# ChristianFeldmann/libHM

Measured on AMD Instinct MI355X. Metric: decoded Mpixels/s (luma), 2160p Main10 reconstruction + loop filters, higher is better.
Workload: dtype int16 samples / int32 accumulate; 1 GPU; 3840x2160 Main10 lowdelay_P pictures, pre-parsed CTU metadata: prep+MC+dequant/IT/recon+deblock+SAO, batch of 16 independent pictures per step, inputs resident in HBM; sub_benchmark=full, streams=2, parallelism=frame-parallel, 1 process per GPU, no data-path collective

## Files before the change

### libhm_amd/csrc/hmgpu_api.hip

```cpp
#include "hmgpu_dev.h"
#include "packed_format.h"

#include <algorithm>
#include <chrono>
#include <atomic>
#include <cstdio>
#include <cstring>
#include <cstdlib>
#include <new>
#include <thread>
#include <unordered_map>
#include <vector>

using namespace hmgpu;

namespace {

enum { K_PREP = 0, K_MC_LUMA, K_MC_CHROMA, K_ITX, K_DBK_VER, K_DBK_HOR, K_SAO, K_EXTEND, K_H2D, K_INTRA, K_FILTER, K_UNPACK };
const char* const kKernelNames[HMGPU_NUM_KERNELS] = {"prep", "mc_luma", "mc_chroma", "itx", "deblock_ver", "deblock_hor", "sao",
                                                     "extend_border", "h2d_stage", "intra", "filter_fused", "unpack"};

struct SliceCall { int first_ctu, num_ctus, slice_idx; bool intra, wp, cells, bi, islice; };

struct Picture {
  bool in_use = false;
  bool sao_applied = false;
  bool filter_ready = false;
  bool sao_any = false;
  bool extended = false;
  std::vector<SliceCall> calls;
  void* planes = nullptr;
  void* meta = nullptr;
  void* coef = nullptr;
  void* pcm = nullptr;
  void* ccp = nullptr;
  void* blob = nullptr;
  void* derived = nullptr;
  uint8_t* sl_table = nullptr;
  uint32_t* coef_start = nullptr;
  std::vector<uint8_t> sl_host;
  PicDev dev;
  std::vector<SliceDev> slices;
  std::vector<SaoDev> h_saoprm;
  std::vector<uint16_t> h_slice_idx, h_tile_idx;
  int max_slice = -1;
  bool flags_staged = true;
  uint64_t last_use = 0;
};

struct EventPair { hipEvent_t a, b; int kind; };

}
// ... 213 lines not shown
    Carver m(pass ? p.meta : nullptr);
    carve_meta(m, p.dev, np, c->num_ctus);
    if (!pass) { HIP_TRY(c, hipMalloc(&p.meta, m.off)); HIP_TRY(c, hipMemset(p.meta, 0, m.off)); }
  }
  {
    size_t bytes = 0;
    for (int k = 0; k < 3; k++) bytes += align_up(c->coef_elems[k] * sizeof(int16_t), 256);
    HIP_TRY(c, hipMalloc(&p.coef, bytes));
    HIP_TRY(c, hipMemset(p.coef, 0, bytes));
    Carver m(p.coef);
    for (int k = 0; k < 3; k++) p.dev.coef[k] = m.take<int16_t>(c->coef_elems[k]);
  }
  for (int pass = 0; pass < 2; pass++) {
    Carver m(pass ? p.derived : nullptr);
    PicDev& d = p.dev;
    d.blk = m.take<BlkInfo>((size_t)c->grid_w * c->grid_h);
    d.edges = m.take<EdgeRec>((size_t)(c->grid_w / 2) * (c->grid_h / 2));
    d.tmv = m.take<TileMv>((size_t)(c->grid_w / 2) * (c->grid_h / 2));
    for (int k = 0; k < 3; k++) d.resid[k] = m.take<int16_t>(c->coef_elems[k]);
    for (int k = 0; k < 3; k++) d.quad_off[k] = m.take<uint32_t>((size_t)c->num_ctus * (c->parts / 4));
    p.coef_start = m.take<uint32_t>((size_t)3 * (c->num_ctus + 1));
    d.fault = m.take<uint32_t>(1);
    for (int k = 0; k < 4; k++) d.tu[k] = m.take<TuRec>((size_t)c->tu_cap[k] * kTuShards);
    d.tu_count = m.take<uint32_t>(4 * kTuShards);
    d.stats = m.take<unsigned long long>(2 * kTuShards);
    d.saoprm = m.take<SaoDev>((size_t)c->num_ctus * 3);
    d.slices = m.take<SliceDev>(HMGPU_MAX_SLICES);
    d.ctu_intra = m.take<uint8_t>((size_t)c->num_ctus);
    p.sl_table = m.take<uint8_t>(4 * 6 * 1024);
    d.intra_done = m.take<uint32_t>((size_t)3 * c->num_ctus);
    if (!pass) { HIP_TRY(c, hipMalloc(&p.derived, m.off)); HIP_TRY(c, hipMemset(p.derived, 0, m.off)); }
  }
  PicDev& d = p.dev;
  d.width = s.width; d.height = s.height;
  d.bd[0] = s.bit_depth_luma; d.bd[1] = d.bd[2] = s.bit_depth_chroma;
  d.log2ctu = s.log2_ctu_size; d.ctus_w = c->ctus_w; d.ctus_h = c->ctus_h; d.num_ctus = c->num_ctus; d.parts = c->parts; d.pw = c->pw;
  for (int k = 0; k < 3; k++) d.pitch[k] = c->pitch[k];
  d.grid_w = c->grid_w; d.grid_h = c->grid_h;
  d.lf_across_tiles = 1; d.sao_applied = 0;
  d.has_intra_dir = 0; d.strong_intra_smoothing = s.strong_intra_smoothing ? 1 : 0;
  d.range_ext = s.range_ext_flags;
  d.mono = s.chroma_format == 0 ? 1 : 0;
  d.fmt = c->fmt; d.csx = c->csx; d.csy = c->csy;
  d.ccp[0] = d.ccp[1] = nullptr;
  d.debug_skip_ctu = -1;
  d.sl_m = nullptr;
  for (int k = 0; k < 3; k++) { d.pcm[k] = nullptr; d.pcm_shift[k] = 0; d.coef_start[k] = nullptr; }
// ... 44 lines not shown
  if (p.extended) return HMGPU_OK;
  Batch b; memset(&b, 0, sizeof(b));
  b.n = 1; b.pic[0] = pic;
  { ProfScope ps(c, K_EXTEND); launch_extend(c->d_pics, b, c->seq.width, c->seq.height, c->mx[0], c->my[0], c->csx, c->csy, c->stream); }
  HIP_TRY(c, hipGetLastError());
  p.extended = true;
  return HMGPU_OK;
}
hmgpu_status ensure_refs_extended(hmgpu_ctx* c, const Batch& b, size_t call_idx) {
  for (int i = 0; i < b.n; i++) {
    const Picture& p = c->pics[b.pic[i]];
    if (call_idx >= p.calls.size()) continue;
    const SliceDev& sd = p.slices[p.calls[call_idx].slice_idx];
    for (int l = 0; l < 2; l++)
      for (int r = 0; r < HMGPU_MAX_REF; r++)
        if (sd.ref_pic[l][r] >= 0) { hmgpu_status st = ensure_extended(c, sd.ref_pic[l][r]); if (st != HMGPU_OK) return st; }
  }
  return HMGPU_OK;
}

hmgpu_status run_recon(hmgpu_ctx* c, const Batch& b, bool any_intra, bool any_wp, bool any_cells, bool any_bi, bool any_islice) {
  int max_ctus = 0;
  for (int i = 0; i < b.n; i++) max_ctus = std::max(max_ctus, b.num_ctus[i]);
  { ProfScope ps(c, K_PREP); launch_prep(c->d_pics, b, max_ctus, c->parts, any_intra, any_cells || c->fmt != 1, c->fmt, c->stream); }
  if (c->fmt != 1) {
    for (int i = 0; i < b.n; i++) {
      const PicDev& d = c->pics[b.pic[i]].dev;
      HIP_TRY(c, hipMemsetAsync(d.resid[1], 0, (size_t)((char*)d.resid[2] - (char*)d.resid[1]) + c->coef_elems[2] * sizeof(int16_t), c->stream));
    }
  }
  McArgs ma;
  memset(&ma, 0, sizeof(ma));
  ma.n = b.n; ma.width = c->seq.width; ma.height = c->seq.height; ma.log2ctu = c->seq.log2_ctu_size; ma.ctus_w = c->ctus_w;
  ma.tw = c->grid_w / 2; ma.npics = c->seq.max_pictures;
  ma.slab = c->plane_slab; ma.pic_stride = 2 * c->plane_bytes; ma.slab_bytes = ma.pic_stride * c->pics.size(); ma.sao_off = (uint32_t)c->plane_bytes;
  for (size_t i = 0; i < c->pics.size(); i++)
    if (c->pics[i].sao_applied) (i < 32 ? ma.sao_mask_lo : ma.sao_mask_hi) |= 1u << (i & 31);
  for (int i = 0; i < b.n; i++) {
    const PicDev& d = c->pics[b.pic[i]].dev;
    ma.first_ctu[i] = b.first_ctu[i]; ma.num_ctus[i] = b.num_ctus[i];
    ma.tmv[i] = d.tmv; ma.slices[i] = d.slices;
  }
  const PicDev& d0 = c->pics[b.pic[0]].dev;
  const char* const base0 = (const char*)c->pics[b.pic[0]].planes;
  uint32_t bps = (uint32_t)std::max(4, std::min(b.n >= 4 ? 12 : 24, max_ctus / 8 + 1));
  {
    ItxArgs ia;
    memset(&ia, 0, sizeof(ia));
    ia.n = b.n; ia.class_mask = 0xf;
    for (int k = 0; k < 3; k++) { ia.rtw[k] = (c->grid_w / 2) >> (k ? c->csx : 0); ia.bd[k] = d0.bd[k]; }
    ia.csx = c->csx; ia.csy = c->csy;
    for (int k = 0; k < 4; k++) ia.tu_cap[k] = c->tu_cap[k];
    for (int i = 0; i < b.n; i++) {
      const PicDev& d = c->pics[b.pic[i]].dev;
      for (int k = 0; k < 4; k++) ia.tu[i][k] = d.tu[k];
      ia.tu_count[i] = d.tu_count;
      for (int k = 0; k < 3; k++) { ia.coef[i][k] = d.coef[k]; ia.resid[i][k] = d.resid[k]; }
      ia.sl_m[i] = d.sl_m;
    }
    ProfScope ps(c, K_ITX);
    launch_itx(ia, bps, c->stream);
    bool any_ccp = false;
    for (int i = 0; i < b.n; i++) any_ccp |= c->pics[b.pic[i]].dev.ccp[0] != nullptr;
    if (any_ccp) launch_ccp(c->d_pics, b, max_ctus, c->stream);
  }
  {
    ProfScope ps(c, K_MC_LUMA);
    ma.pitch = c->pitch[0]; ma.bd = c->seq.bit_depth_luma;
    ma.origin_off = (uint32_t)((const char*)d0.rec[0] - base0);
    ma.rtw = c->grid_w / 2;
    for (int i = 0; i < b.n; i++) { ma.dst[i] = c->pics[b.pic[i]].dev.rec[0]; ma.resid[i] = c->pics[b.pic[i]].dev.resid[0]; }
    launch_mc_luma(ma, max_ctus, any_wp, any_bi, c->stream);
    if (any_cells) launch_mc_luma_cells(c->d_pics, c->d_finals, b, max_ctus, c->seq.log2_ctu_size, any_wp, c->stream);
  }
  if (c->fmt != 1) {
    ProfScope ps(c, K_MC_CHROMA);
    launch_mc_chroma_fmt(c->d_pics, c->d_finals, b, max_ctus, c->seq.log2_ctu_size, c->fmt, any_wp, c->stream);
  } else if (c->seq.chroma_format != 0) {
    ProfScope ps(c, K_MC_CHROMA);
// ... 1568 lines not shown
```

### libhm_amd/csrc/hmgpu_dev.h

```cpp
#pragma once
#include <hip/hip_runtime.h>
#include <stdint.h>
#include "../../include/hmgpu.h"

namespace hmgpu {

constexpr int kMaxBatch = 16;
constexpr int kMaxPics = 64;
constexpr int kTuShards = 8;
constexpr int kCStep = 2;

struct __attribute__((aligned(16))) BlkInfo {
  int16_t mv[2][2];
  int8_t  ref[2];
  int8_t  qp;
  uint8_t flags;
  uint8_t edge;
  uint8_t log2cu;
  uint16_t slice;
};
static_assert(sizeof(BlkInfo) == 16, "BlkInfo must be 16 bytes");

enum : uint8_t {
  BF_VALID = 1,
// ... 131 lines not shown
  const SliceDev* slices[kMaxBatch];
  const char* slab;
  uint64_t pic_stride, slab_bytes;
  uint32_t sao_off, origin_off, cr_off;
  uint32_t sao_mask_lo, sao_mask_hi;
};

struct ItxArgs {
  int32_t n; uint32_t class_mask;
  int32_t blocks[4];
  int32_t rtw[3], bd[3];
  int32_t csx, csy;
  uint32_t tu_cap[4];
  const TuRec* tu[kMaxBatch][4];
  const uint32_t* tu_count[kMaxBatch];
  const int16_t* coef[kMaxBatch][3];
  int16_t* resid[kMaxBatch][3];
  const uint8_t* sl_m[kMaxBatch];
};

#define HMGPU_AS1 __attribute__((address_space(1)))
typedef uint32_t u32x4 __attribute__((ext_vector_type(4)));
typedef uint32_t u32x2 __attribute__((ext_vector_type(2)));
typedef u32x4 u32x4_a8 __attribute__((aligned(8)));
template <typename T> __device__ inline T ldg(const T* p) { return *(const T HMGPU_AS1*)p; }
template <typename T> __device__ inline void stg(T* p, T v) { *(T HMGPU_AS1*)p = v; }
__device__ inline u32x4 ldg4(const void* p) { return *(const u32x4 HMGPU_AS1*)p; }
__device__ inline u32x4 ldg4_a8(const void* p) { return *(const u32x4_a8 HMGPU_AS1*)p; }
__device__ inline u32x2 ldg2(const void* p) { return *(const u32x2 HMGPU_AS1*)p; }
__device__ inline void stg4(void* p, u32x4 v) { *(u32x4 HMGPU_AS1*)p = v; }
__device__ inline void stg4_a8(void* p, u32x4 v) { *(u32x4_a8 HMGPU_AS1*)p = v; }
__device__ inline void stg2(void* p, u32x2 v) { *(u32x2 HMGPU_AS1*)p = v; }

__host__ __device__ inline int zscan_x(int z) {
  int x = z & 0x5555; x = (x | (x >> 1)) & 0x3333; x = (x | (x >> 2)) & 0x0f0f; x = (x | (x >> 4)) & 0x00ff; return x;
}
__host__ __device__ inline int zscan_y(int z) { return zscan_x(z >> 1); }
__device__ inline int clip3(int lo, int hi, int v) { return min(hi, max(lo, v)); }
__device__ inline BlkInfo ld_blk(const BlkInfo* p) { return __builtin_bit_cast(BlkInfo, ldg4(p)); }

__device__ inline bool xcd_remap(int bid, int n, int nb, int& slot, int& lb) {
  if (n < 0) { n = -n; slot = bid % n; lb = bid / n; return lb < nb; }
  if (n <= 8 && (8 % n) == 0) {
    const int m = 8 / n;
    const int per = (nb + m - 1) / m;
    const int x = bid & 7, t = bid >> 3;
    slot = x % n;
    const int r = x / n;
    lb = r * per + t;
    return t < per && lb < nb;
  }
  slot = bid % n; lb = bid / n;
  return lb < nb;
}
__host__ inline int xcd_grid(int n, int nb) {
  if (n <= 8 && (8 % n) == 0) { const int m = 8 / n; return 8 * ((nb + m - 1) / m); }
  return n * nb;
}

struct UnpackArgs {
  int32_t n;
  int32_t pic[kMaxBatch];
  const char* blob[kMaxBatch];
};
void launch_unpack_input(const PicDev* pics, const UnpackArgs& ua, int num_ctus, hipStream_t s);
void launch_prep(const PicDev* pics, const Batch& b, int max_ctus, int parts, bool intra, bool write_blk, int fmt, hipStream_t s);
void launch_mc_luma(McArgs& a, int max_ctus, bool wp, bool bi, hipStream_t s);
void launch_mc_chroma(McArgs& a, int max_ctus, bool wp, bool bi, hipStream_t s);
void launch_mc_luma_cells(const PicDev* pics, const PlaneSet* finals, const Batch& b, int max_ctus, int log2ctu, bool wp, hipStream_t s);
void launch_mc_chroma_cells(const PicDev* pics, const PlaneSet* finals, const Batch& b, int max_ctus, int log2ctu, bool wp, hipStream_t s);
void launch_itx(ItxArgs& a, uint32_t blocks_per_shard, hipStream_t s);
void launch_filter_fused(const PicDev* pics, const Batch& b, int width, int height, bool nofilt, hipStream_t s);
void launch_pack(const int16_t* src, int pitch, int step, int x0, int y0, int w, int h, int bytes, uint8_t* dst, int dst_stride, hipStream_t s);
void launch_unpack(const int16_t* src, int w, int h, int16_t* dst, int pitch, int step, hipStream_t s);
void launch_checksum(const int16_t* src, int pitch, int step, int w, int h, int bd, uint32_t* out, hipStream_t s);
struct Md5Batch { int32_t n, pad_; const uint8_t* msg[128]; unsigned long long bytes[128]; uint32_t* out[128]; };
void launch_md5(const Md5Batch& job, hipStream_t s);
void launch_crc(const int16_t* src, int pitch, int step, int w, int h, int bd, uint32_t* rows, uint32_t* out, hipStream_t s);
void launch_intra(const PicDev* pics, const Batch& b, const int32_t* order, int num_ctus, bool lean, hipStream_t s);
struct ExportArgs {
  const int16_t* y;
  const int16_t* c;
  int32_t pitch_y, pitch_c;
  int32_t layout, bytes, mono, csx, csy;
  int32_t w, h, cw, ch;
  int32_t sh[2], maxv[2];
  int32_t msb[2];
  int32_t vec;
  uint8_t* dst[3];
// ... 18 lines not shown
```

### libhm_amd/csrc/k_prep.hip

```cpp
#include "hmgpu_dev.h"
#include "filter_core.h"

namespace hmgpu {

__constant__ uint8_t c_chroma_scale_420[58] = {
    0, 1, 2, 3, 4, 5, 6, 7, 8, 9, 10, 11, 12, 13, 14, 15, 16, 17, 18, 19, 20, 21, 22, 23, 24, 25, 26, 27, 28, 29,
    29, 30, 31, 32, 33, 33, 34, 34, 35, 35, 36, 36, 37, 37, 38, 39, 40, 41, 42, 43, 44, 45, 46, 47, 48, 49, 50, 51};

__constant__ uint8_t c_chroma422_mode[36] = {
    0, 1, 2, 2, 2, 2, 3, 5, 7, 8, 10, 12, 13, 15, 17, 18, 19, 20, 21, 22, 23, 23, 24, 24, 25, 25, 26, 27, 27, 28, 28, 29, 29, 30, 31, 36};

__device__ inline void qp_param(int qp_y, int comp, int bd, int chroma_off, int fmt, int8_t& per, int8_t& rem) {
  const int bdo = 6 * (bd - 8);
  int base;
  if (comp == 0) base = qp_y + bdo;
  else {
    base = clip3(-bdo, 57, qp_y + chroma_off);
    base = base < 0 ? base + bdo : (fmt == 1 ? c_chroma_scale_420[base] : min(base, 51)) + bdo;
  }
  per = (int8_t)(base / 6);
  rem = (int8_t)(base % 6);
}

struct Quad {
  int ctu, z0, gx0, gy0;
  int log2cu, log2tu, tr, part_size, qp_cu, sidx;
  bool valid, intra;
  uint32_t cbf[3], ts[3];
  uint32_t bypass;
};

__device__ inline TuRec make_tu(const PicDev& P, const Quad& q, const SliceDev* sl, int gx, int gy, int comp, int flags, int xflags, uint32_t coef_off) {
  TuRec r;
  r.x4 = (uint16_t)gx; r.y4 = (uint16_t)gy;
  r.comp_flags = (uint8_t)(comp | (flags << 2));
  const int coff = comp == 1 ? ldg(&sl->cb_qp_offset) : (comp == 2 ? ldg(&sl->cr_qp_offset) : 0);
  qp_param(q.qp_cu, comp, P.bd[comp], coff, P.fmt, r.per, r.rem);
  r.xflags = (uint8_t)xflags;
  r.coef_off = coef_off;
  return r;
}

__device__ inline int z_of(int x, int y) {
  int z = 0;
#pragma unroll
  for (int k = 0; k < 4; k++) z |= (((x >> k) & 1) << (2 * k)) | (((y >> k) & 1) << (2 * k + 1));
  return z;
}

__device__ inline BlkInfo cell_from_arrays(const PicDev& P, int ctu, int z) {
  BlkInfo bi;
  bi.mv[0][0] = bi.mv[0][1] = bi.mv[1][0] = bi.mv[1][1] = 0;
  bi.ref[0] = bi.ref[1] = -1;
  bi.qp = 0; bi.flags = 0; bi.edge = 0; bi.log2cu = 3; bi.slice = 0;
  const size_t i = (size_t)ctu * P.parts + z;
  if ((int)ldg(P.part_size + i) == HMGPU_SIZE_NONE) return bi;
  const int sidx = P.slice_idx ? ldg(P.slice_idx + ctu) : 0;
  const SliceDev* sl = P.slices + sidx;
  const int tr = ldg(P.tr_idx + i);
  const bool intra = ldg(P.pred_mode + i) == HMGPU_MODE_INTRA;
  bi.flags = BF_VALID | (intra ? BF_INTRA : 0) | (((ldg(P.cbf[0] + i) >> tr) & 1) ? BF_CBFY : 0);
  if (ldg(P.bypass + i) || (P.pcm_lf_disable && ldg(P.ipcm + i))) bi.flags |= BF_NOFILT;
  bi.qp = ldg(P.qp + i);
  bi.log2cu = (uint8_t)(P.log2ctu - ldg(P.depth + i));
  bi.slice = (uint16_t)sidx;
  if (!intra) {
    const int r0 = ldg(P.ref_idx[0] + i), r1 = ldg(P.ref_idx[1] + i);
    if (r0 >= 0) { const uint32_t w = ldg(reinterpret_cast<const uint32_t*>(P.mv[0]) + i); bi.mv[0][0] = (int16_t)(w & 0xffff); bi.mv[0][1] = (int16_t)(w >> 16); bi.ref[0] = ldg(&sl->ref_pic[0][r0]); }
    if (r1 >= 0 && ldg(&sl->slice_type) == HMGPU_B_SLICE) { const uint32_t w = ldg(reinterpret_cast<const uint32_t*>(P.mv[1]) + i); bi.mv[1][0] = (int16_t)(w & 0xffff); bi.mv[1][1] = (int16_t)(w >> 16); bi.ref[1] = ldg(&sl->ref_pic[1][r1]); }
  }
  return bi;
}

__device__ inline uint16_t edge_unit(const BlkInfo& p, const BlkInfo& q, bool transform_edge) {
  const int bs = boundary_strength(p, q, transform_edge);
  if (bs == 0) return 0;
  return (uint16_t)edge_unit_pack(bs, ((int)p.qp + (int)q.qp + 1) >> 1, (p.flags & BF_NOFILT) != 0, (q.flags & BF_NOFILT) != 0);
}

template <int FMT>
__global__ void __launch_bounds__(256) k_prep(const PicDev* __restrict__ pics, Batch b, int write_blk) {
  constexpr int NS = FMT == 1 ? 6 : 12;
  __shared__ uint32_t lds_cnt[4], lds_base[4], lds_stat[2];
  __shared__ __attribute__((aligned(16))) u32x4 lds_cell[256 * 4];
  __shared__ __attribute__((aligned(16))) u32x4 lds_above[256], lds_left[16];
  const PicDev& P = pics[b.pic[blockIdx.z]];
  if (threadIdx.x < 4) lds_cnt[threadIdx.x] = 0;
  if (threadIdx.x < 2) lds_stat[threadIdx.x] = 0;
  __syncthreads();
  const int parts = P.parts;
#if defined(PREP_STOP) && PREP_STOP == 1
  if (parts > 0) return;
#endif
  const int gq = blockIdx.x * 256 + threadIdx.x;
  const bool active = gq < b.num_ctus[blockIdx.z] * (parts >> 2);
  Quad q; q.valid = false; q.intra = false; q.log2tu = 3; q.tr = 0; q.ctu = 0; q.z0 = 0; q.gx0 = q.gy0 = 0;
  q.log2cu = 3; q.part_size = 0; q.qp_cu = 0; q.sidx = 0; q.bypass = 0;
  uint32_t hasm = 0;
  auto set_has = [&](int k, bool v) { hasm |= (v ? 1u : 0u) << k; };
  auto has = [&](int k) { return ((hasm >> k) & 1u) != 0; };
  uint32_t cnt[3] = {0, 0, 0}, lmask = 0;
  int cls[NS] = {};
  uint32_t loc[NS] = {};
  const SliceDev* sl = P.slices;
  u32x4 cells[4] = {{0, 0, 0, 0}, {0, 0, 0, 0}, {0, 0, 0, 0}, {0, 0, 0, 0}};
  write_blk |= P.any_nofilt;
  if (active) {
    q.ctu = b.first_ctu[blockIdx.z] + gq / (parts >> 2);
    q.z0 = (gq % (parts >> 2)) * 4;
    const size_t idx = (size_t)q.ctu * parts + q.z0;
    const int cx = q.ctu % P.ctus_w, cy = q.ctu / P.ctus_w;
    const int x4 = zscan_x(q.z0), y4 = zscan_y(q.z0);
    q.gx0 = cx * P.pw + x4; q.gy0 = cy * P.pw + y4;
    {
      const int qpc = parts >> 2, lane_c = q.z0 >> 2, t0 = (int)threadIdx.x - lane_c, cl = t0 / qpc, pw = P.pw;
      const bool need_above = cy > 0 && t0 - P.ctus_w * qpc < 0, need_left = cx > 0 && t0 - qpc < 0;
#pragma unroll 1
      for (int r = lane_c; r < 2 * pw; r += qpc) {
        const bool left = r >= pw;
        const int i = left ? r - pw : r;
#if defined(PREP_EXP) && (PREP_EXP & 1)
        if (false) {
#else
        if (left ? need_left : need_above) {
#endif
          const u32x4 v = __builtin_bit_cast(u32x4, cell_from_arrays(P, left ? q.ctu - 1 : q.ctu - P.ctus_w, left ? z_of(pw - 1, i) : z_of(i, pw - 1)));
          if (left) lds_left[i] = v; else lds_above[cl * pw + i] = v;
        }
      }
    }
#if defined(PREP_STOP) && PREP_STOP == 2
    if (parts > 0) return;
#endif
    const uint32_t part4 = ldg(reinterpret_cast<const uint32_t*>(P.part_size + idx));
    const uint32_t depth4 = ldg(reinterpret_cast<const uint32_t*>(P.depth + idx));
    const uint32_t pred4 = ldg(reinterpret_cast<const uint32_t*>(P.pred_mode + idx));
    const uint32_t qp4 = ldg(reinterpret_cast<const uint32_t*>(P.qp + idx));
    const uint32_t tr4 = ldg(reinterpret_cast<const uint32_t*>(P.tr_idx + idx));
    const uint32_t byp4 = ldg(reinterpret_cast<const uint32_t*>(P.bypass + idx)), pcm4 = ldg(reinterpret_cast<const uint32_t*>(P.ipcm + idx));
    const uint32_t r04 = ldg(reinterpret_cast<const uint32_t*>(P.ref_idx[0] + idx)), r14 = ldg(reinterpret_cast<const uint32_t*>(P.ref_idx[1] + idx));
    const u32x4 mv0 = ldg4(P.mv[0] + idx * 2), mv1 = ldg4(P.mv[1] + idx * 2);
#pragma unroll
    for (int c = 0; c < 3; c++) {
      q.cbf[c] = ldg(reinterpret_cast<const uint32_t*>(P.cbf[c] + idx));
      q.ts[c] = P.tskip[c] ? ldg(reinterpret_cast<const uint32_t*>(P.tskip[c] + idx)) : 0u;
    }
    q.bypass = byp4;
    q.sidx = P.slice_idx ? ldg(P.slice_idx + q.ctu) : 0;
    sl = P.slices + q.sidx;
    q.part_size = (int)(int8_t)(part4 & 0xff);
    const int px0 = q.gx0 * 4, py0 = q.gy0 * 4;
    q.valid = px0 < P.width && py0 < P.height && q.part_size != HMGPU_SIZE_NONE;
    const int depth = depth4 & 0xff;
    q.tr = tr4 & 0xff;
    q.log2cu = P.log2ctu - depth;
    q.log2tu = q.log2cu - q.tr;
    q.intra = (pred4 & 0xff) == HMGPU_MODE_INTRA;
    const int cu_parts = 1 << (q.log2cu - 2);
    q.qp_cu = (int)ldg(P.qp + (size_t)q.ctu * parts + (q.z0 & ~(cu_parts * cu_parts - 1)));
    const int tu_parts = q.log2tu > 2 ? 1 << (q.log2tu - 2) : 1;
    const bool deblock = q.valid && !ldg(&sl->deblocking_disable);
    const int lf_across_slices = ldg(&sl->lf_across_slices);
    const int slice_type = ldg(&sl->slice_type);
    const bool wp = ldg(&sl->weighted_pred) != 0;
#if defined(PREP_STOP) && PREP_STOP == 3
    if (parts > 0) {
      if ((part4 ^ depth4 ^ pred4 ^ qp4 ^ tr4 ^ byp4 ^ pcm4 ^ r04 ^ r14 ^ mv0.x ^ mv1.w ^ q.cbf[0] ^ q.cbf[1] ^ q.cbf[2] ^ q.ts[0] ^ (uint32_t)q.qp_cu ^ (uint32_t)deblock ^
           (uint32_t)lf_across_slices ^ (uint32_t)slice_type ^ (uint32_t)wp) == 0x12345677u) stg(P.tu_count, 1u);
      return;
    }
#endif
    const uint32_t mvw0[4] = {mv0.x, mv0.y, mv0.z, mv0.w}, mvw1[4] = {mv1.x, mv1.y, mv1.z, mv1.w};
    uint32_t tm_mv[4][2], tm_key[4];
#pragma unroll
    for (int j = 0; j < 4; j++) {
      const int xj = x4 + (j & 1), yj = y4 + (j >> 1);
      const int gx = q.gx0 + (j & 1), gy = q.gy0 + (j >> 1);
      BlkInfo bi;
      bi.mv[0][0] = bi.mv[0][1] = bi.mv[1][0] = bi.mv[1][1] = 0;
      bi.ref[0] = bi.ref[1] = -1;
      bi.qp = 0; bi.flags = 0; bi.edge = 0; bi.log2cu = 3; bi.slice = 0;
      if (q.valid) {
        const int cbf_y = (q.cbf[0] >> (8 * j)) & 0xff;
        bi.flags = BF_VALID | (q.intra ? BF_INTRA : 0) | (((cbf_y >> q.tr) & 1) ? BF_CBFY : 0);
        if (((byp4 >> (8 * j)) & 0xff) || (P.pcm_lf_disable && ((pcm4 >> (8 * j)) & 0xff))) bi.flags |= BF_NOFILT;
        bi.qp = (int8_t)((qp4 >> (8 * j)) & 0xff);
        bi.log2cu = (uint8_t)q.log2cu;
        bi.slice = (uint16_t)q.sidx;
        if (!q.intra) {
          const int r0 = (int)(int8_t)((r04 >> (8 * j)) & 0xff), r1 = (int)(int8_t)((r14 >> (8 * j)) & 0xff);
          int use0 = r0 >= 0, use1 = r1 >= 0 && slice_type == HMGPU_B_SLICE;
// ... 108 lines not shown
      if (q.log2tu > 2) {
        const int tu_parts2 = 1 << (q.log2tu - 2);
        if ((x4 & (tu_parts2 - 1)) == 0 && (y4 & (tu_parts2 - 1)) == 0) {
          if (((q.cbf[0] & 0xff) & chain) == chain) cnt[0] = 1u << (2 * q.log2tu);
          if (((q.cbf[1] & 0xff) & chain) == chain) cnt[1] = 1u << (2 * q.log2tu - 2);
          if (((q.cbf[2] & 0xff) & chain) == chain) cnt[2] = 1u << (2 * q.log2tu - 2);
        }
      } else {
#pragma unroll
        for (int j = 0; j < 4; j++) if ((((q.cbf[0] >> (8 * j)) & 0xff) & chain) == chain) lmask |= 1u << j;
        cnt[0] = 16u * __popc(lmask);
        if (((q.cbf[1] & 0xff) & chain) == chain) cnt[1] = 16;
        if (((q.cbf[2] & 0xff) & chain) == chain) cnt[2] = 16;
      }
    }
#if defined(PREP_STOP) && PREP_STOP == 4
    if (parts > 0) return;
#endif
    if (q.valid) atomicAdd(&lds_stat[q.intra ? 0 : 1], 4u);
    {
      const int qpc = parts >> 2, ln = threadIdx.x & 63, seg = ln & ~(qpc - 1);
      const unsigned long long m = __builtin_amdgcn_ballot_w64(q.valid && q.intra);
      const unsigned long long sm = qpc >= 64 ? m : (m >> seg) & ((1ull << qpc) - 1ull);
      if (ln == seg && sm) stg(P.ctu_intra + q.ctu, (uint8_t)__popcll(sm));
    }
    if (q.valid && q.log2tu <= 5 && (!q.intra || (P.has_intra_dir && !(pcm4 & 0xff)))) {
      const uint32_t chain = (1u << (q.tr + 1)) - 1;
      if (q.log2tu > 2) {
        const int tu_parts = 1 << (q.log2tu - 2);
        if ((x4 & (tu_parts - 1)) == 0 && (y4 & (tu_parts - 1)) == 0) {
          set_has(0, ((q.cbf[0] & 0xff) & chain) == chain); cls[0] = q.log2tu - 2;
          if constexpr (FMT == 1) {
            set_has(4, ((q.cbf[1] & 0xff) & chain) == chain); cls[4] = q.log2tu - 3;
            set_has(5, ((q.cbf[2] & 0xff) & chain) == chain); cls[5] = q.log2tu - 3;
          } else {
#pragma unroll
            for (int c = 1; c < 3; c++) {
              set_has(4 * c, ((q.cbf[c] & 0xff) & chain) == chain); cls[4 * c] = FMT == 3 ? q.log2tu - 2 : q.log2tu - 3;
              if constexpr (FMT == 2) { set_has(4 * c + 1, has(4 * c)); cls[4 * c + 1] = cls[4 * c]; }
            }
          }
        }
      } else {
#pragma unroll
        for (int j = 0; j < 4; j++) { set_has(j, (((q.cbf[0] >> (8 * j)) & 0xff) & chain) == chain); cls[j] = 0; }
        if constexpr (FMT == 1) {
          set_has(4, ((q.cbf[1] & 0xff) & chain) == chain); cls[4] = 0;
// ... 18 lines not shown
#pragma unroll
    for (int c = 0; c < 3; c++) {
      uint32_t incl = cnt[c];
#pragma unroll
      for (int d = 1; d < 64; d <<= 1) { const uint32_t o = __shfl_up(incl, d); if (lane >= d) incl += o; }
      const uint32_t excl = incl - cnt[c];
      const uint32_t seg = __shfl(excl, lane & ~(qpc - 1));
      coff[c] = excl - seg;
      if (active) {
        coff[c] += ldg(P.coef_start[c] + q.ctu);
        stg(P.quad_off[c] + (size_t)q.ctu * qpc + (q.z0 >> 2), coff[c]);
      }
    }
  }
#if defined(PREP_STOP) && PREP_STOP == 5
  if (parts > 0) return;
#endif
#if !(defined(PREP_EXP) && (PREP_EXP & 4))
  if (active) {
#pragma unroll
    for (int j = 0; j < 4; j++) lds_cell[threadIdx.x * 4 + j] = cells[j];
  }
#endif
  __syncthreads();
  if (active) {
    EdgeRec er; er.v[0] = er.v[1] = er.h[0] = er.h[1] = 0;
#if defined(PREP_EXP) && (PREP_EXP & 2)
    if (false) {
#else
    if (q.valid) {
#endif
      const int x4 = zscan_x(q.z0), y4 = zscan_y(q.z0), qpc = parts >> 2;
      const int t0 = (int)threadIdx.x - (q.z0 >> 2);
#pragma unroll
      for (int k = 0; k < 2; k++) {
        {
          const BlkInfo Q = __builtin_bit_cast(BlkInfo, cells[2 * k]);
          if (Q.edge & BE_VER_FILTER) {
            BlkInfo Pn;
            if (x4 > 0) Pn = __builtin_bit_cast(BlkInfo, lds_cell[(t0 + (z_of(x4 - 2, y4) >> 2)) * 4 + 2 * k + 1]);
            else {
              const int tn = t0 - qpc + (z_of(P.pw - 2, y4) >> 2);
              if (tn >= 0) Pn = __builtin_bit_cast(BlkInfo, lds_cell[tn * 4 + 2 * k + 1]);
              else Pn = __builtin_bit_cast(BlkInfo, lds_left[y4 + k]);
            }
            er.v[k] = edge_unit(Pn, Q, (Q.edge & BE_VER_TRANSFORM) != 0);
          }
        }
        {
          const BlkInfo Q = __builtin_bit_cast(BlkInfo, cells[k]);
          if (Q.edge & BE_HOR_FILTER) {
            BlkInfo Pn;
            if (y4 > 0) Pn = __builtin_bit_cast(BlkInfo, lds_cell[(t0 + (z_of(x4, y4 - 2) >> 2)) * 4 + 2 + k]);
            else {
              const int tn = t0 - P.ctus_w * qpc + (z_of(x4, P.pw - 2) >> 2);
              if (tn >= 0) Pn = __builtin_bit_cast(BlkInfo, lds_cell[tn * 4 + 2 + k]);
              else Pn = __builtin_bit_cast(BlkInfo, lds_above[(t0 / qpc) * P.pw + x4 + k]);
            }
            er.h[k] = edge_unit(Pn, Q, (Q.edge & BE_HOR_TRANSFORM) != 0);
          }
        }
      }
    }
    stg2(reinterpret_cast<uint32_t*>(P.edges + (size_t)(q.gy0 >> 1) * (P.grid_w >> 1) + (q.gx0 >> 1)), __builtin_bit_cast(u32x2, er));
  }
#if defined(PREP_STOP) && PREP_STOP == 6
  if (parts > 0) return;
#endif
  const int shard = blockIdx.x & (kTuShards - 1);
  if (threadIdx.x < 4) {
    const uint32_t n = lds_cnt[threadIdx.x];
    lds_base[threadIdx.x] = n ? atomicAdd(&P.tu_count[threadIdx.x * kTuShards + shard], n) : 0u;
  } else if (threadIdx.x < 6) {
    const uint32_t n = lds_stat[threadIdx.x - 4];
    if (n) atomicAdd(&P.stats[(threadIdx.x - 4) * kTuShards + shard], (unsigned long long)n);
  }
  __syncthreads();
#if defined(PREP_STOP) && PREP_STOP == 7
  if (parts > 0) return;
#endif
  const int ctu_luma = 1 << (2 * P.log2ctu);
#pragma unroll
  for (int k = 0; k < NS; k++) {
    if (!has(k)) continue;
    const int comp = FMT == 1 ? (k < 4 ? 0 : k - 3) : k >> 2;
    int j = FMT == 1 ? (k < 4 ? k : 0) : (k & 3), dx = j & 1, dy = j >> 1, bsize = comp == 0 ? q.log2tu : max(q.log2tu - 1, 2);
    int ts = (q.ts[comp] >> (8 * j)) & 0xff;
    uint32_t off = comp == 0 ? (uint32_t)q.ctu * ctu_luma + 16u * (q.z0 + j) : (uint32_t)q.ctu * (ctu_luma >> 2) + 4u * q.z0;
    if constexpr (FMT == 3) {
      bsize = q.log2tu;
      off = (uint32_t)q.ctu * ctu_luma + 16u * (q.z0 + j);
    } else if constexpr (FMT == 2) {
      if (comp) {
        const int l2 = max(q.log2tu, 3) - 1, n = 1 << l2, lower = j;
        bsize = l2; dx = 0; dy = lower ? n >> 2 : 0;
        off = (uint32_t)q.ctu * (ctu_luma >> 1) + 8u * q.z0 + (lower ? (uint32_t)(n * n) : 0u);
        ts = !lower ? (q.ts[comp] & 0xff) : q.log2tu <= 3 ? (q.ts[comp] >> 16) & 0xff : (P.tskip[comp] ? (int)ldg(P.tskip[comp] + (size_t)q.ctu * P.parts + q.z0 + (1 << (2 * (q.log2tu - 2) - 1))) : 0);
        j = 0;
      }
    }
    int flags = ((comp == 0 && q.log2tu == 2 && q.intra) ? 1 : 0) | ((ts & 1) ? 2 : 0) | ((q.bypass & 0xff) ? 4 : 0) | (q.intra ? 32 : 0);
    int xflags = 0;
    if ((flags & 6) && P.range_ext) {
      if (!q.intra) {
        if (P.range_ext & HMGPU_REXT_EXPLICIT_RDPCM) flags |= ((ts >> 1) & 3) << 3;
      } else {
        if ((P.range_ext & HMGPU_REXT_ROTATION) && bsize == 2) xflags |= 1;
        if (P.range_ext & HMGPU_REXT_IMPLICIT_RDPCM) {
          const size_t cb = (size_t)q.ctu * P.parts;
          int mode = ldg(P.intra_dir[comp ? 1 : 0] + cb + q.z0 + j);
          if (comp && mode == 36) mode = ldg(P.intra_dir[0] + cb + (FMT == 3 ? q.z0 + j : (q.z0 & ~((1 << (2 * (q.log2cu - 2))) - 1))));
          if (FMT == 2 && comp) mode = c_chroma422_mode[mode];
          flags |= (mode == 10 ? 1 : mode == 26 ? 2 : 0) << 3;
        }
      }
    }
    if (FMT == 1 && P.coef_start[0] != nullptr) off = coff[comp] + (comp == 0 ? 16u * __popc(lmask & ((1u << j) - 1u)) : 0u);
    const TuRec r = make_tu(P, q, sl, q.gx0 + dx, q.gy0 + dy, comp, flags, xflags, off);
    const int c = cls[k];
    const uint32_t i = lds_base[c] + loc[k];
    if (i < P.tu_cap[c]) {
      uint32_t* dst = reinterpret_cast<uint32_t*>(P.tu[c] + (size_t)shard * P.tu_cap[c] + i);
      const uint32_t* src = reinterpret_cast<const uint32_t*>(&r);
      stg(dst, src[0]); stg(dst + 1, src[1]); stg(dst + 2, src[2]);
    }
  }
}

__global__ void k_zero_counts(const PicDev* __restrict__ pics, Batch b, int intra) {
  const PicDev& P = pics[b.pic[blockIdx.x]];
  if (threadIdx.x < 4 * kTuShards) stg(P.tu_count + threadIdx.x, 0u);
  for (int i = threadIdx.x; i < b.num_ctus[blockIdx.x]; i += blockDim.x) stg(P.ctu_intra + b.first_ctu[blockIdx.x] + i, (uint8_t)0);
  if (intra) for (int i = threadIdx.x; i < 3 * P.num_ctus; i += blockDim.x) stg(P.intra_done + i, 0u);
}

void launch_prep(const PicDev* pics, const Batch& b, int max_ctus, int parts, bool intra, bool write_blk, int fmt, hipStream_t s) {
  hipLaunchKernelGGL(k_zero_counts, dim3((unsigned)b.n), dim3(256), 0, s, pics, b, intra ? 1 : 0);
  dim3 grid((unsigned)(((size_t)max_ctus * (parts / 4) + 255) / 256), 1, (unsigned)b.n);
  if (fmt == 3) hipLaunchKernelGGL(k_prep<3>, grid, dim3(256), 0, s, pics, b, write_blk ? 1 : 0);
  else if (fmt == 2) hipLaunchKernelGGL(k_prep<2>, grid, dim3(256), 0, s, pics, b, write_blk ? 1 : 0);
  else hipLaunchKernelGGL(k_prep<1>, grid, dim3(256), 0, s, pics, b, write_blk ? 1 : 0);
}

}
```

Baseline: 175,600 Mpixels/s.

## Fuse count zeroing into prep kernel with double-buffered TU counters and wave-local neighbors

```diff
diff --git a/libhm_amd/csrc/hmgpu_api.hip b/libhm_amd/csrc/hmgpu_api.hip
--- a/libhm_amd/csrc/hmgpu_api.hip
+++ b/libhm_amd/csrc/hmgpu_api.hip
@@ -28,6 +28,7 @@
   bool filter_ready = false;
   bool sao_any = false;
   bool extended = false;
+  uint32_t tu_count_set = 0;
   std::vector<SliceCall> calls;
   void* planes = nullptr;
   void* meta = nullptr;
@@ -287,7 +288,7 @@
     p.coef_start = m.take<uint32_t>((size_t)3 * (c->num_ctus + 1));
     d.fault = m.take<uint32_t>(1);
     for (int k = 0; k < 4; k++) d.tu[k] = m.take<TuRec>((size_t)c->tu_cap[k] * kTuShards);
-    d.tu_count = m.take<uint32_t>(4 * kTuShards);
+    d.tu_count = m.take<uint32_t>(2 * 4 * kTuShards);
     d.stats = m.take<unsigned long long>(2 * kTuShards);
     d.saoprm = m.take<SaoDev>((size_t)c->num_ctus * 3);
     d.slices = m.take<SliceDev>(HMGPU_MAX_SLICES);
@@ -378,7 +379,10 @@
 hmgpu_status run_recon(hmgpu_ctx* c, const Batch& b, bool any_intra, bool any_wp, bool any_cells, bool any_bi, bool any_islice) {
   int max_ctus = 0;
   for (int i = 0; i < b.n; i++) max_ctus = std::max(max_ctus, b.num_ctus[i]);
-  { ProfScope ps(c, K_PREP); launch_prep(c->d_pics, b, max_ctus, c->parts, any_intra, any_cells || c->fmt != 1, c->fmt, c->stream); }
+  uint32_t cnt_sel = 0;
+  for (int i = 0; i < b.n; i++) cnt_sel |= c->pics[b.pic[i]].tu_count_set << i;
+  { ProfScope ps(c, K_PREP); launch_prep(c->d_pics, b, max_ctus, c->parts, any_intra, any_cells || c->fmt != 1, c->fmt, cnt_sel, c->stream); }
+  for (int i = 0; i < b.n; i++) c->pics[b.pic[i]].tu_count_set ^= 1u;
   if (c->fmt != 1) {
     for (int i = 0; i < b.n; i++) {
       const PicDev& d = c->pics[b.pic[i]].dev;
@@ -410,7 +414,7 @@
     for (int i = 0; i < b.n; i++) {
       const PicDev& d = c->pics[b.pic[i]].dev;
       for (int k = 0; k < 4; k++) ia.tu[i][k] = d.tu[k];
-      ia.tu_count[i] = d.tu_count;
+      ia.tu_count[i] = d.tu_count + ((cnt_sel >> i) & 1u) * (4 * kTuShards);
       for (int k = 0; k < 3; k++) { ia.coef[i][k] = d.coef[k]; ia.resid[i][k] = d.resid[k]; }
       ia.sl_m[i] = d.sl_m;
     }
diff --git a/libhm_amd/csrc/hmgpu_dev.h b/libhm_amd/csrc/hmgpu_dev.h
--- a/libhm_amd/csrc/hmgpu_dev.h
+++ b/libhm_amd/csrc/hmgpu_dev.h
@@ -177,6 +177,8 @@
 #define HMGPU_AS1 __attribute__((address_space(1)))
 typedef uint32_t u32x4 __attribute__((ext_vector_type(4)));
 typedef uint32_t u32x2 __attribute__((ext_vector_type(2)));
+typedef uint32_t u32x3 __attribute__((ext_vector_type(3)));
+typedef u32x3 u32x3_a4 __attribute__((aligned(4)));
 typedef u32x4 u32x4_a8 __attribute__((aligned(8)));
 template <typename T> __device__ inline T ldg(const T* p) { return *(const T HMGPU_AS1*)p; }
 template <typename T> __device__ inline void stg(T* p, T v) { *(T HMGPU_AS1*)p = v; }
@@ -186,6 +188,7 @@
 __device__ inline void stg4(void* p, u32x4 v) { *(u32x4 HMGPU_AS1*)p = v; }
 __device__ inline void stg4_a8(void* p, u32x4 v) { *(u32x4_a8 HMGPU_AS1*)p = v; }
 __device__ inline void stg2(void* p, u32x2 v) { *(u32x2 HMGPU_AS1*)p = v; }
+__device__ inline void stg3_a4(void* p, u32x3 v) { *(u32x3_a4 HMGPU_AS1*)p = v; }
 
 __host__ __device__ inline int zscan_x(int z) {
   int x = z & 0x5555; x = (x | (x >> 1)) & 0x3333; x = (x | (x >> 2)) & 0x0f0f; x = (x | (x >> 4)) & 0x00ff; return x;
@@ -219,7 +222,7 @@
   const char* blob[kMaxBatch];
 };
 void launch_unpack_input(const PicDev* pics, const UnpackArgs& ua, int num_ctus, hipStream_t s);
-void launch_prep(const PicDev* pics, const Batch& b, int max_ctus, int parts, bool intra, bool write_blk, int fmt, hipStream_t s);
+void launch_prep(const PicDev* pics, const Batch& b, int max_ctus, int parts, bool intra, bool write_blk, int fmt, uint32_t cnt_sel, hipStream_t s);
 void launch_mc_luma(McArgs& a, int max_ctus, bool wp, bool bi, hipStream_t s);
 void launch_mc_chroma(McArgs& a, int max_ctus, bool wp, bool bi, hipStream_t s);
 void launch_mc_luma_cells(const PicDev* pics, const PlaneSet* finals, const Batch& b, int max_ctus, int log2ctu, bool wp, hipStream_t s);
diff --git a/libhm_amd/csrc/k_prep.hip b/libhm_amd/csrc/k_prep.hip
--- a/libhm_amd/csrc/k_prep.hip
+++ b/libhm_amd/csrc/k_prep.hip
@@ -3,12 +3,10 @@
 
 namespace hmgpu {
 
-__constant__ uint8_t c_chroma_scale_420[58] = {
-    0, 1, 2, 3, 4, 5, 6, 7, 8, 9, 10, 11, 12, 13, 14, 15, 16, 17, 18, 19, 20, 21, 22, 23, 24, 25, 26, 27, 28, 29,
-    29, 30, 31, 32, 33, 33, 34, 34, 35, 35, 36, 36, 37, 37, 38, 39, 40, 41, 42, 43, 44, 45, 46, 47, 48, 49, 50, 51};
-
 __constant__ uint8_t c_chroma422_mode[36] = {
     0, 1, 2, 2, 2, 2, 3, 5, 7, 8, 10, 12, 13, 15, 17, 18, 19, 20, 21, 22, 23, 23, 24, 24, 25, 25, 26, 27, 27, 28, 28, 29, 29, 30, 31, 36};
+
+__device__ inline int chroma_scale_420(int i) { return i < 30 ? i : i < 34 ? i - 1 : i < 44 ? 33 + ((i - 34) >> 1) : i - 6; }
 
 __device__ inline void qp_param(int qp_y, int comp, int bd, int chroma_off, int fmt, int8_t& per, int8_t& rem) {
   const int bdo = 6 * (bd - 8);
@@ -16,7 +14,7 @@
   if (comp == 0) base = qp_y + bdo;
   else {
     base = clip3(-bdo, 57, qp_y + chroma_off);
-    base = base < 0 ? base + bdo : (fmt == 1 ? c_chroma_scale_420[base] : min(base, 51)) + bdo;
+    base = base < 0 ? base + bdo : (fmt == 1 ? chroma_scale_420(base) : min(base, 51)) + bdo;
   }
   per = (int8_t)(base / 6);
   rem = (int8_t)(base % 6);
@@ -30,15 +28,9 @@
   uint32_t bypass;
 };
 
-__device__ inline TuRec make_tu(const PicDev& P, const Quad& q, const SliceDev* sl, int gx, int gy, int comp, int flags, int xflags, uint32_t coef_off) {
-  TuRec r;
-  r.x4 = (uint16_t)gx; r.y4 = (uint16_t)gy;
-  r.comp_flags = (uint8_t)(comp | (flags << 2));
-  const int coff = comp == 1 ? ldg(&sl->cb_qp_offset) : (comp == 2 ? ldg(&sl->cr_qp_offset) : 0);
-  qp_param(q.qp_cu, comp, P.bd[comp], coff, P.fmt, r.per, r.rem);
-  r.xflags = (uint8_t)xflags;
-  r.coef_off = coef_off;
-  return r;
+__device__ inline u32x3 make_tu(int gx, int gy, int comp, int flags, int xflags, uint32_t perrem, uint32_t coef_off) {
+  return (u32x3){(uint32_t)(uint16_t)gx | ((uint32_t)(uint16_t)gy << 16),
+                 (uint32_t)(uint8_t)(comp | (flags << 2)) | (perrem << 8) | ((uint32_t)(uint8_t)xflags << 24), coef_off};
 }
 
 __device__ inline int z_of(int x, int y) {
@@ -47,6 +39,10 @@
   for (int k = 0; k < 4; k++) z |= (((x >> k) & 1) << (2 * k)) | (((y >> k) & 1) << (2 * k + 1));
   return z;
 }
+
+constexpr int kMortonX = 0x5555, kMortonY = 0xaaaa;
+__device__ inline int area_left(int a) { return (((a & kMortonX) - 1) & kMortonX) | (a & kMortonY); }
+__device__ inline int area_above(int a) { return (((a & kMortonY) - 1) & kMortonY) | (a & kMortonX); }
 
 __device__ inline BlkInfo cell_from_arrays(const PicDev& P, int ctu, int z) {
   BlkInfo bi;
@@ -79,21 +75,26 @@
 }
 
 template <int FMT>
-__global__ void __launch_bounds__(256) k_prep(const PicDev* __restrict__ pics, Batch b, int write_blk) {
+__global__ void __launch_bounds__(256) k_prep(const PicDev* __restrict__ pics, Batch b, int write_blk, uint32_t cnt_sel, int intra) {
   constexpr int NS = FMT == 1 ? 6 : 12;
   __shared__ uint32_t lds_cnt[4], lds_base[4], lds_stat[2];
   __shared__ __attribute__((aligned(16))) u32x4 lds_cell[256 * 4];
-  __shared__ __attribute__((aligned(16))) u32x4 lds_above[256], lds_left[16];
+  __shared__ __attribute__((aligned(16))) u32x4 lds_above[256], lds_left[4 * 16];
   const PicDev& P = pics[b.pic[blockIdx.z]];
+  const uint32_t sel = (cnt_sel >> blockIdx.z) & 1u;
+  uint32_t* const tu_count = P.tu_count + sel * (4 * kTuShards);
+  if (blockIdx.x == 0 && threadIdx.x < 4 * kTuShards) stg(P.tu_count + (sel ^ 1u) * (4 * kTuShards) + threadIdx.x, 0u);
+  if (intra)
+    for (int i = blockIdx.x * 256 + threadIdx.x; i < 3 * P.num_ctus; i += gridDim.x * 256) stg(P.intra_done + i, 0u);
   if (threadIdx.x < 4) lds_cnt[threadIdx.x] = 0;
   if (threadIdx.x < 2) lds_stat[threadIdx.x] = 0;
   __syncthreads();
-  const int parts = P.parts;
+  const int parts = P.parts, lq = 2 * P.log2ctu - 6;
 #if defined(PREP_STOP) && PREP_STOP == 1
   if (parts > 0) return;
 #endif
   const int gq = blockIdx.x * 256 + threadIdx.x;
-  const bool active = gq < b.num_ctus[blockIdx.z] * (parts >> 2);
+  const bool active = gq < (b.num_ctus[blockIdx.z] << lq);
   Quad q; q.valid = false; q.intra = false; q.log2tu = 3; q.tr = 0; q.ctu = 0; q.z0 = 0; q.gx0 = q.gy0 = 0;
   q.log2cu = 3; q.part_size = 0; q.qp_cu = 0; q.sidx = 0; q.bypass = 0;
   uint32_t hasm = 0;
@@ -106,15 +107,15 @@
   u32x4 cells[4] = {{0, 0, 0, 0}, {0, 0, 0, 0}, {0, 0, 0, 0}, {0, 0, 0, 0}};
   write_blk |= P.any_nofilt;
   if (active) {
-    q.ctu = b.first_ctu[blockIdx.z] + gq / (parts >> 2);
-    q.z0 = (gq % (parts >> 2)) * 4;
+    q.ctu = b.first_ctu[blockIdx.z] + (gq >> lq);
+    q.z0 = (gq & ((1 << lq) - 1)) * 4;
     const size_t idx = (size_t)q.ctu * parts + q.z0;
     const int cx = q.ctu % P.ctus_w, cy = q.ctu / P.ctus_w;
     const int x4 = zscan_x(q.z0), y4 = zscan_y(q.z0);
     q.gx0 = cx * P.pw + x4; q.gy0 = cy * P.pw + y4;
     {
-      const int qpc = parts >> 2, lane_c = q.z0 >> 2, t0 = (int)threadIdx.x - lane_c, cl = t0 / qpc, pw = P.pw;
-      const bool need_above = cy > 0 && t0 - P.ctus_w * qpc < 0, need_left = cx > 0 && t0 - qpc < 0;
+      const int qpc = parts >> 2, lane_c = q.z0 >> 2, t0 = (int)threadIdx.x - lane_c, tw = t0 & 63, pw = P.pw;
+      const bool need_above = cy > 0 && tw - P.ctus_w * qpc < 0, need_left = cx > 0 && tw - qpc < 0;
 #pragma unroll 1
       for (int r = lane_c; r < 2 * pw; r += qpc) {
         const bool left = r >= pw;
@@ -125,7 +126,7 @@
         if (left ? need_left : need_above) {
 #endif
           const u32x4 v = __builtin_bit_cast(u32x4, cell_from_arrays(P, left ? q.ctu - 1 : q.ctu - P.ctus_w, left ? z_of(pw - 1, i) : z_of(i, pw - 1)));
-          if (left) lds_left[i] = v; else lds_above[cl * pw + i] = v;
+          if (left) lds_left[(threadIdx.x >> 6) * 16 + i] = v; else lds_above[(t0 >> lq) * pw + i] = v;
         }
       }
     }
@@ -166,7 +167,7 @@
 #if defined(PREP_STOP) && PREP_STOP == 3
     if (parts > 0) {
       if ((part4 ^ depth4 ^ pred4 ^ qp4 ^ tr4 ^ byp4 ^ pcm4 ^ r04 ^ r14 ^ mv0.x ^ mv1.w ^ q.cbf[0] ^ q.cbf[1] ^ q.cbf[2] ^ q.ts[0] ^ (uint32_t)q.qp_cu ^ (uint32_t)deblock ^
-           (uint32_t)lf_across_slices ^ (uint32_t)slice_type ^ (uint32_t)wp) == 0x12345677u) stg(P.tu_count, 1u);
+           (uint32_t)lf_across_slices ^ (uint32_t)slice_type ^ (uint32_t)wp) == 0x12345677u) stg(tu_count, 1u);
       return;
     }
 #endif
@@ -321,7 +322,7 @@
       const int qpc = parts >> 2, ln = threadIdx.x & 63, seg = ln & ~(qpc - 1);
       const unsigned long long m = __builtin_amdgcn_ballot_w64(q.valid && q.intra);
       const unsigned long long sm = qpc >= 64 ? m : (m >> seg) & ((1ull << qpc) - 1ull);
-      if (ln == seg && sm) stg(P.ctu_intra + q.ctu, (uint8_t)__popcll(sm));
+      if (ln == seg) stg(P.ctu_intra + q.ctu, (uint8_t)__popcll(sm));
     }
     if (q.valid && q.log2tu <= 5 && (!q.intra || (P.has_intra_dir && !(pcm4 & 0xff)))) {
       const uint32_t chain = (1u << (q.tr + 1)) - 1;
@@ -386,7 +387,9 @@
     for (int j = 0; j < 4; j++) lds_cell[threadIdx.x * 4 + j] = cells[j];
   }
 #endif
-  __syncthreads();
+  __builtin_amdgcn_fence(__ATOMIC_RELEASE, "wavefront");
+  __builtin_amdgcn_wave_barrier();
+  __builtin_amdgcn_fence(__ATOMIC_ACQUIRE, "wavefront");
   if (active) {
     EdgeRec er; er.v[0] = er.v[1] = er.h[0] = er.h[1] = 0;
 #if defined(PREP_EXP) && (PREP_EXP & 2)
@@ -394,20 +397,18 @@
 #else
     if (q.valid) {
 #endif
-      const int x4 = zscan_x(q.z0), y4 = zscan_y(q.z0), qpc = parts >> 2;
-      const int t0 = (int)threadIdx.x - (q.z0 >> 2);
+      const int x4 = zscan_x(q.z0), y4 = zscan_y(q.z0), qpc = parts >> 2, a = q.z0 >> 2;
+      const int t0 = (int)threadIdx.x - a, tw = t0 & 63;
+      const int above_off = P.ctus_w * qpc;
 #pragma unroll
       for (int k = 0; k < 2; k++) {
         {
           const BlkInfo Q = __builtin_bit_cast(BlkInfo, cells[2 * k]);
           if (Q.edge & BE_VER_FILTER) {
             BlkInfo Pn;
-            if (x4 > 0) Pn = __builtin_bit_cast(BlkInfo, lds_cell[(t0 + (z_of(x4 - 2, y4) >> 2)) * 4 + 2 * k + 1]);
-            else {
-              const int tn = t0 - qpc + (z_of(P.pw - 2, y4) >> 2);
-              if (tn >= 0) Pn = __builtin_bit_cast(BlkInfo, lds_cell[tn * 4 + 2 * k + 1]);
-              else Pn = __builtin_bit_cast(BlkInfo, lds_left[y4 + k]);
-            }
+            if (x4 > 0) Pn = __builtin_bit_cast(BlkInfo, lds_cell[(t0 + area_left(a)) * 4 + 2 * k + 1]);
+            else if (tw >= qpc) Pn = __builtin_bit_cast(BlkInfo, lds_cell[(t0 - qpc + ((kMortonX & (qpc - 1)) | a)) * 4 + 2 * k + 1]);
+            else Pn = __builtin_bit_cast(BlkInfo, lds_left[(threadIdx.x >> 6) * 16 + y4 + k]);
             er.v[k] = edge_unit(Pn, Q, (Q.edge & BE_VER_TRANSFORM) != 0);
           }
         }
@@ -415,12 +416,9 @@
           const BlkInfo Q = __builtin_bit_cast(BlkInfo, cells[k]);
           if (Q.edge & BE_HOR_FILTER) {
             BlkInfo Pn;
-            if (y4 > 0) Pn = __builtin_bit_cast(BlkInfo, lds_cell[(t0 + (z_of(x4, y4 - 2) >> 2)) * 4 + 2 + k]);
-            else {
-              const int tn = t0 - P.ctus_w * qpc + (z_of(x4, P.pw - 2) >> 2);
-              if (tn >= 0) Pn = __builtin_bit_cast(BlkInfo, lds_cell[tn * 4 + 2 + k]);
-              else Pn = __builtin_bit_cast(BlkInfo, lds_above[(t0 / qpc) * P.pw + x4 + k]);
-            }
+            if (y4 > 0) Pn = __builtin_bit_cast(BlkInfo, lds_cell[(t0 + area_above(a)) * 4 + 2 + k]);
+            else if (tw >= above_off) Pn = __builtin_bit_cast(BlkInfo, lds_cell[(t0 - above_off + ((kMortonY & (qpc - 1)) | a)) * 4 + 2 + k]);
+            else Pn = __builtin_bit_cast(BlkInfo, lds_above[(t0 >> lq) * P.pw + x4 + k]);
             er.h[k] = edge_unit(Pn, Q, (Q.edge & BE_HOR_TRANSFORM) != 0);
           }
         }
@@ -431,10 +429,11 @@
 #if defined(PREP_STOP) && PREP_STOP == 6
   if (parts > 0) return;
 #endif
+  __syncthreads();
   const int shard = blockIdx.x & (kTuShards - 1);
   if (threadIdx.x < 4) {
     const uint32_t n = lds_cnt[threadIdx.x];
-    lds_base[threadIdx.x] = n ? atomicAdd(&P.tu_count[threadIdx.x * kTuShards + shard], n) : 0u;
+    lds_base[threadIdx.x] = n ? atomicAdd(&tu_count[threadIdx.x * kTuShards + shard], n) : 0u;
   } else if (threadIdx.x < 6) {
     const uint32_t n = lds_stat[threadIdx.x - 4];
     if (n) atomicAdd(&P.stats[(threadIdx.x - 4) * kTuShards + shard], (unsigned long long)n);
@@ -443,7 +442,15 @@
 #if defined(PREP_STOP) && PREP_STOP == 7
   if (parts > 0) return;
 #endif
+  if (!hasm) return;
   const int ctu_luma = 1 << (2 * P.log2ctu);
+  uint32_t perrem[3];
+#pragma unroll
+  for (int c = 0; c < 3; c++) {
+    int8_t per, rem;
+    qp_param(q.qp_cu, c, P.bd[c], c == 1 ? ldg(&sl->cb_qp_offset) : (c == 2 ? ldg(&sl->cr_qp_offset) : 0), P.fmt, per, rem);
+    perrem[c] = (uint32_t)(uint8_t)per | ((uint32_t)(uint8_t)rem << 8);
+  }
 #pragma unroll
   for (int k = 0; k < NS; k++) {
     if (!has(k)) continue;
@@ -480,30 +487,18 @@
       }
     }
     if (FMT == 1 && P.coef_start[0] != nullptr) off = coff[comp] + (comp == 0 ? 16u * __popc(lmask & ((1u << j) - 1u)) : 0u);
-    const TuRec r = make_tu(P, q, sl, q.gx0 + dx, q.gy0 + dy, comp, flags, xflags, off);
     const int c = cls[k];
     const uint32_t i = lds_base[c] + loc[k];
-    if (i < P.tu_cap[c]) {
-      uint32_t* dst = reinterpret_cast<uint32_t*>(P.tu[c] + (size_t)shard * P.tu_cap[c] + i);
-      const uint32_t* src = reinterpret_cast<const uint32_t*>(&r);
-      stg(dst, src[0]); stg(dst + 1, src[1]); stg(dst + 2, src[2]);
-    }
-  }
-}
-
-__global__ void k_zero_counts(const PicDev* __restrict__ pics, Batch b, int intra) {
-  const PicDev& P = pics[b.pic[blockIdx.x]];
-  if (threadIdx.x < 4 * kTuShards) stg(P.tu_count + threadIdx.x, 0u);
-  for (int i = threadIdx.x; i < b.num_ctus[blockIdx.x]; i += blockDim.x) stg(P.ctu_intra + b.first_ctu[blockIdx.x] + i, (uint8_t)0);
-  if (intra) for (int i = threadIdx.x; i < 3 * P.num_ctus; i += blockDim.x) stg(P.intra_done + i, 0u);
-}
-
-void launch_prep(const PicDev* pics, const Batch& b, int max_ctus, int parts, bool intra, bool write_blk, int fmt, hipStream_t s) {
-  hipLaunchKernelGGL(k_zero_counts, dim3((unsigned)b.n), dim3(256), 0, s, pics, b, intra ? 1 : 0);
+    if (i < P.tu_cap[c]) stg3_a4(P.tu[c] + (size_t)shard * P.tu_cap[c] + i, make_tu(q.gx0 + dx, q.gy0 + dy, comp, flags, xflags, perrem[comp], off));
+  }
+}
+
+void launch_prep(const PicDev* pics, const Batch& b, int max_ctus, int parts, bool intra, bool write_blk, int fmt, uint32_t cnt_sel, hipStream_t s) {
   dim3 grid((unsigned)(((size_t)max_ctus * (parts / 4) + 255) / 256), 1, (unsigned)b.n);
-  if (fmt == 3) hipLaunchKernelGGL(k_prep<3>, grid, dim3(256), 0, s, pics, b, write_blk ? 1 : 0);
-  else if (fmt == 2) hipLaunchKernelGGL(k_prep<2>, grid, dim3(256), 0, s, pics, b, write_blk ? 1 : 0);
-  else hipLaunchKernelGGL(k_prep<1>, grid, dim3(256), 0, s, pics, b, write_blk ? 1 : 0);
-}
-
-}
+  const int wb = write_blk ? 1 : 0, in = intra ? 1 : 0;
+  if (fmt == 3) hipLaunchKernelGGL(k_prep<3>, grid, dim3(256), 0, s, pics, b, wb, cnt_sel, in);
+  else if (fmt == 2) hipLaunchKernelGGL(k_prep<2>, grid, dim3(256), 0, s, pics, b, wb, cnt_sel, in);
+  else hipLaunchKernelGGL(k_prep<1>, grid, dim3(256), 0, s, pics, b, wb, cnt_sel, in);
+}
+
+}
```

Measured after the change: 176,900 Mpixels/s, median of 6. About the same (+0.7%).
